# zyansheep/shadow

Hardware: AMD Instinct MI355X
Metric: APSP routing build (s) @10k nodes; packets routed/sec per sim round (lower is better)
Workload: dtype u64+f32; 1 GPU; C3 APSP routing build: 10k-node undirected ring+chords graph, mean degree 8, latency U[1,100] ms (integer us), loss 0 w.p. 0.8 else U(0,0.02); all nodes used; source rows sharded across ranks (each rank keeps its row block; the optional RCCL all-gather of the blocks is timed separately in apsp_detail.allgather_ms); nodes=10000, arcs=79996, parallelism=rows1

## Files before the change

shadow_amd/csrc/sg_routing.hip:

```cpp
#include <algorithm>
#include <cstring>
#include <string>
#include <vector>

#include "sg_device.h"
#include "sg_internal.h"
#include "sg_knobs.h"

namespace sg {

__global__ void k_self_check(const uint32_t* __restrict__ used, uint32_t n_used,
                             const uint32_t* __restrict__ self_cnt,
                             unsigned long long* __restrict__ first) {
  for (uint32_t j = blockIdx.x * blockDim.x + threadIdx.x; j < n_used; j += gridDim.x * blockDim.x) {
    uint32_t c = self_cnt[used[j]];
    if (c != 1) atomicMin(first, ((unsigned long long)j << 1) | (c > 1 ? 1ull : 0ull));
  }
}

__global__ void __launch_bounds__(1024) k_build_finish(const uint32_t* __restrict__ sat, uint32_t rows,
                                                       const uint32_t* __restrict__ used, uint32_t n_used,
                                                       const uint32_t* __restrict__ self_cnt, uint32_t* __restrict__ ret,
                                                       int count_flags) {
  constexpr int G = 8;
// ... 321 lines not shown
  for (uint32_t r = 0; r < n_diag; r++) {
    for (int k = 0; k < DW; k++) a[k] += (double)h[(size_t)r * DW + k];
    const unsigned long long w3 = h[(size_t)r * DW + 3];
    setup += (double)(w3 >> 24);
    a[3] -= (double)(w3 >> 22 << 22);
    if (h[(size_t)r * DW] == 0) continue;
    const int c = (int)((w3 >> 22) & 1);
    cn[c] += 1;
    cs[c] += (double)(w3 >> 24);
    cq[c] += (double)h[(size_t)r * DW];
  }
  for (int c = 0; c < 2; c++)
    fprintf(stderr, "[sssp] %s rows: %.0f, mean setup %.0f cyc, mean search %.0f cyc\n", c ? "chained" : "unchained",
            cn[c], cs[c] / std::max(1.0, cn[c]), cq[c] / std::max(1.0, cn[c]));
  fprintf(stderr, "[sssp] mean setup (init + bound rows) %.0f cyc of the search\n", setup / n_diag);
  fprintf(stderr, "[sssp] setup parts: bound-row listing and load issue %.0f, LDS pass %.0f, barrier %.0f, first load "
          "round %.0f, later rounds and closing barrier %.0f cyc\n", a[9] / n_diag, a[8] / n_diag, a[10] / n_diag,
          a[11] / n_diag, a[12] / n_diag);
  fprintf(stderr, "[sssp] per-wave cycles summed over a row's 16 waves: claim+wait %.0f, pop %.0f, steps %.0f "
          "(per pop: %.0f, %.0f)\n", a[5] / n_diag, a[6] / n_diag, a[7] / n_diag, a[6] / std::max(1.0, a[2]),
          a[7] / std::max(1.0, a[2]));
  fprintf(stderr, "[sssp] delta %u ns, %u rows: mean search %.0f cyc, output %.0f cyc, %.1f wave pops, %.1f buckets, "
          "%.0f relaxations (%.2f x arcs)\n", delta, n_diag, a[0] / n_diag, a[1] / n_diag, a[2] / n_diag,
          a[3] / n_diag, a[4] / n_diag, a[4] / n_diag / std::max(1u, net->n_arcs));
}

static void shortest_paths_lds(sg_ctx* ctx, sg_net* net, const uint32_t* d_used, uint32_t n_used, uint32_t row_begin,
                               uint32_t row_end, uint64_t* out_lat, float* out_loss) {
  hipStream_t st = ctx->stream;
  const uint32_t rows = row_end - row_begin;
  const LdsKnobs k = lds_knobs(ctx, net, n_used, rows);
  *(volatile uint32_t*)(ctx->apsp_ret + 4) = 0u;
  bool told = false;
// ... 484 lines not shown
```

shadow_amd/csrc/sg_sssp.hip:

```cpp
#include <algorithm>
#include <cstdlib>
#include <type_traits>

#include "sg_device.h"
#include "sg_internal.h"
#include "sg_knobs.h"

namespace sg {

constexpr int SSSP_THREADS = 1024;
constexpr int SSSP_WAVES = SSSP_THREADS / 64;
constexpr int SSSP_K = 4;
constexpr int SSSP_KB = SSSP_KB_MAX;
constexpr size_t SSSP_STATIC_LDS = 4 * (8 + SSSP_WAVES) + 16 + SSSP_WAVES * 64 * SSSP_K + 512 + 4 * (3 * SSSP_KB + 1) + 16;

constexpr size_t LDS_PER_CU = 160 * 1024;

constexpr uint64_t FKEY_INF = ((uint64_t)LAT32_SAT << 32) | ((uint64_t)0x3F800000u << 1);
__device__ __forceinline__ uint32_t fkey_lat(uint64_t k) { return (uint32_t)(k >> 32); }
__device__ __forceinline__ uint32_t fkey_loss_bits(uint64_t k) { return ((uint32_t)k >> 1) & 0x7FFFFFFFu; }
__device__ __forceinline__ uint64_t frelax(uint64_t ku, uint32_t edge_lat, float edge_om) {
  const uint32_t lat = __builtin_elementwise_add_sat(fkey_lat(ku), edge_lat);
  const float loss = fold_loss(__uint_as_float(fkey_loss_bits(ku)), edge_om);
  return ((uint64_t)lat << 32) | (uint32_t)((__float_as_uint(loss) << 1) | 1u);
// ... 89 lines not shown
    const __amdgpu_buffer_rsrc_t ro = __builtin_amdgcn_make_buffer_rsrc((void*)out_off, 0, (int)((n + 1) * 4u),
                                                                        0x00020000);
    constexpr int GO = 12;
    for (uint32_t v0 = tid; v0 <= n; v0 += GO * NT) {
      uint32_t to[GO];
#pragma unroll
      for (int g = 0; g < GO; g++) {
        const uint32_t v = v0 + g * NT;
        to[g] = __builtin_amdgcn_raw_buffer_load_b32(ro, v <= n ? v * 4u : OOB, 0, 0);
      }
#pragma unroll
      for (int g = 0; g < GO; g++)
        if (v0 + g * NT <= n) off[v0 + g * NT] = to[g];
    }
  }
  __shared__ uint32_t s_item;
  __shared__ uint32_t s_chain, s_cw, s_psat;
  auto next_listed = [&]() -> uint32_t {
    uint32_t* claim_w = chain_on ? chain_args()->claim : nullptr;
    for (;;) {
      const uint32_t b = atomicAdd(item_ctr, 1u);
      if (!claim_w || b >= n_items) return b;
      const uint32_t r = blk_rows ? blk_rows[b] : row_begin + b;
      if (atomicCAS(&claim_w[r - row_begin], 0u, 1u) == 0u) return b;
    }
  };
  for (uint32_t i = tid; i < cap; i += NT) ring[i] = RING_EMPTY;
  for (int i = tid; i < NW * 64 * SSSP_K; i += NT) (&own[0][0])[i] = 0;
  if (pop_diag && tid < SSSP_POP_WORDS) s_popc[tid] = 0ull;
  if (item_ctr && tid == 0) {
    s_item = next_listed();
    s_chain = 0u;
    s_psat = 0u;
  }
  for (uint32_t it = 0;; it++) {
    uint32_t bi, chain = 0, chain_w = 0;
    if (item_ctr) {
      __syncthreads();
      bi = s_item;
      if (bi >= n_items) break;
      if (chain_on) {
        chain = s_chain;
        chain_w = s_cw;
        if (chain > 1u && !(chain_args()->exact && !s_psat)) chain = 1u;
      }
    } else {
      if (it) break;
      bi = blockIdx.x;
      if (bi >= n_items) break;
// ... 27 lines not shown
      }
      if (lane == 0) s_nub = (uint32_t)__popcll(mk);
    };
    int nb = 0;
    if (ub_row && (FLAG ? tid < 64 : it == 0)) list_bounds(bi);
    if (ub_row) {
      if constexpr (FLAG) {
        __syncthreads();
      } else {
        __builtin_amdgcn_fence(__ATOMIC_RELEASE, "wavefront");
        __builtin_amdgcn_wave_barrier();
        __builtin_amdgcn_fence(__ATOMIC_ACQUIRE, "wavefront");
      }
      nb = (int)s_nub;
    }
    unsigned long long c_list = 0, c_init = 0, c_bar = 0, c_g0 = 0;
    auto lds_pass = [&]() {
      if (dg) c_list = clock64();
      if (chain) {
        const bool ex = (chain & 2u) != 0;
        for (uint32_t v = tid; v < n; v += NT) {
          const uint64_t kv = key[v];
          const uint64_t lw = (uint64_t)fkey_lat(kv) + chain_w;
          uint64_t nk = FKEY_INF;
          if (fkey_lat(kv) != LAT32_SAT && lw < LAT32_SAT - 1)
            nk = ex ? (lw << 32) | ((uint32_t)kv & ~1u) : ((lw + 1) << 32) | ((uint64_t)0x3F800000u << 1);
          key[v] = nk;
        }
        if (COUNT && tid == 0) {
          atomicAdd(&work[WORK_SHARDS], 1ull);
          if (ex) atomicAdd(&work[WORK_SHARDS + 1], 1ull);
        }
      } else {
        for (uint32_t v = tid; v < n; v += NT) key[v] = FKEY_INF;
      }
      if (tid < 8) ctl[tid] = 0;
      if (tid == 0) hb = 0;
      if (dg) c_init = clock64();
      __syncthreads();
      if (dg) c_bar = clock64();
    };
    if (!nb) {
      lds_pass();
    } else {
      constexpr int GC = 10;
      const __amdgpu_buffer_rsrc_t ru = __builtin_amdgcn_make_buffer_rsrc((void*)used, 0, (int)(n_used * 4u),
                                                                          0x00020000);
      int k = 0;
      uint32_t jb = 0;
      uint32_t ts = (uint32_t)tid;
      asm volatile("" : "+v"(ts));
#pragma unroll 1
      do {
        const uint32_t j0 = jb + ts;
        uint32_t vv[GC];
        uint64_t l[2][GC];
        uint32_t f[2][GC];
        bool on[2], exact[2];
        uint32_t sr[2];
#pragma unroll
        for (int u = 0; u < 2; u++) {
          on[u] = k + u < nb;
          sr[u] = on[u] ? __builtin_amdgcn_readfirstlane(s_ub[k + u][0]) : 0u;
          exact[u] = on[u] && __builtin_amdgcn_readfirstlane(s_ub[k + u][2]);
          const size_t rb = on[u] ? (size_t)(sr[u] - out_row0) * n_used : 0;
          const __amdgpu_buffer_rsrc_t rl =
              __builtin_amdgcn_make_buffer_rsrc((void*)(out_lat + rb), 0, (int)(on[u] ? n_used * 8u : 0u), 0x00020000);
          const __amdgpu_buffer_rsrc_t rf = __builtin_amdgcn_make_buffer_rsrc(
// ... 43 lines not shown
      } while (k < nb);
    }
    if (ub_row) __syncthreads();
    const unsigned long long c_setup = dg ? clock64() : 0;
    if (tid == 0) {
      key[src] = 1ull;
      ring[0] = (uint16_t)src;
      ctl[TAIL] = 1;
      s_psat = 0u;
    }
    uint32_t split = delta;
    const __amdgpu_buffer_rsrc_t arcs = __builtin_amdgcn_make_buffer_rsrc((void*)out_arc, 0, (int)(n_arcs * 12u),
                                                                          0x00020000);
    uint32_t n_rel = 0;
    const uint32_t max_adv = 4u * n + 64u;
    uint8_t* ow = own[wv];
    uint32_t spins = 0;
    constexpr int ABORT = 2;
    auto give_up = [&]() {
      if (lane == 0) {
        sat_row[row - row_begin] = 2u;
        *any_flag = 1u;
        if (atomicExch(&ctl[ABORT], 1u) == 0u && item_ctr) {
          __threadfence();
          if (atomicAdd(&item_ctr[1], 1u) == gridDim.x - 1) {
            const uint32_t c = __hip_atomic_load(&item_ctr[0], __ATOMIC_RELAXED, __HIP_MEMORY_SCOPE_AGENT);
            uint32_t* claim_w = chain_on ? chain_args()->claim : nullptr;
            for (uint32_t i = min(c, n_items); i < n_items; i++) {
              const uint32_t r = (blk_rows ? blk_rows[i] : row_begin + i) - row_begin;
              if (!claim_w || __hip_atomic_load(&claim_w[r], __ATOMIC_RELAXED, __HIP_MEMORY_SCOPE_AGENT) == 0u)
                sat_row[r] = 2u;
            }
          }
// ... 8 lines not shown
#pragma unroll
      for (int c = 0; c < NK; c++) {
        const bool ok = valid[c] && fkey_lat(cand[c]) != LAT32_SAT;
        okk[c] = ok;
        cd[c] = cand[c];
        old[c] = __hip_atomic_fetch_min(ok ? &key[v[c]] : &sink[lane], (unsigned long long)cd[c], __ATOMIC_RELAXED,
                                        __HIP_MEMORY_SCOPE_WORKGROUP);
      }
      __builtin_amdgcn_sched_barrier(0);
#pragma unroll
      for (int c = 0; c < NK; c++)
        app[c] = __builtin_amdgcn_ballot_w64(okk[c] && !((uint32_t)old[c] & 1u) && old[c] > cd[c] &&
                                             fkey_lat(cd[c]) < split);
    };
    __syncthreads();

    for (;;) {
      const unsigned long long tc0 = (COUNT && diag) ? clock64() : 0;
      uint32_t h = 0, k = 0;
      if (lane == 0) {
        for (;;) {
          const unsigned long long w = __hip_atomic_load(&hb, __ATOMIC_RELAXED, __HIP_MEMORY_SCOPE_WORKGROUP);
          const uint32_t hh = (uint32_t)(w >> 32), t = ld(&ctl[TAIL]);
          if (t == hh) break;
          const uint32_t kk = min(claim, t - hh);
          const unsigned long long nw = ((unsigned long long)(hh + kk) << 32) | ((w & 0xFFFFFFFFull) + 1);
          if (atomicCAS(&hb, w, nw) == w) {
            h = hh;
            k = kk;
            break;
          }
        }
      }
      h = __builtin_amdgcn_readfirstlane(h);
      k = __builtin_amdgcn_readfirstlane(k);
      if (__builtin_amdgcn_readfirstlane(ld(&ctl[ABORT]))) goto wave_exit;
      if (!k) {
        uint32_t q = 0;
        if (lane == 0) {
          const unsigned long long w = __hip_atomic_load(&hb, __ATOMIC_RELAXED, __HIP_MEMORY_SCOPE_WORKGROUP);
          __atomic_signal_fence(__ATOMIC_SEQ_CST);
          q = (w & 0xFFFFFFFFull) == 0 && (uint32_t)(w >> 32) == ld(&ctl[TAIL]);
        }
        if (!__builtin_amdgcn_readfirstlane(q)) {
          if (++spins > spin_max) {
            give_up();
            goto wave_exit;
          }
          for (uint32_t z = 0; z < idle_sleep; z++) __builtin_amdgcn_s_sleep(8);
          __builtin_amdgcn_s_sleep(2);
          continue;
        }
        __syncthreads();
        if (ld(&ctl[ABORT])) goto wave_exit;
        if (split >= LAT32_SAT) break;
        uint32_t m = LAT32_SAT;
        for (uint32_t v = tid; v < n; v += NT) {
          const uint64_t kv = key[v];
          if (kv & 1ull) m = min(m, fkey_lat(kv));
        }
        for (int d = 32; d > 0; d >>= 1) m = min(m, (uint32_t)__shfl_xor(m, d));
        if (lane == 0) red[wv] = m;
        __syncthreads();
        m = red[0];
        for (int w = 1; w < NW; w++) m = min(m, red[w]);
        if (m == LAT32_SAT) break;
        if (++n_adv > max_adv) {
          give_up();
          goto wave_exit;
        }
        split = m + delta >= m ? min(m + delta, LAT32_SAT) : LAT32_SAT;
        for (uint32_t v0 = wv * 64; v0 < n; v0 += NT) {
          const uint32_t v = v0 + lane;
          uint64_t kv = v < n ? key[v] : 0ull;
          const bool q2 = (kv & 1ull) && fkey_lat(kv) < split;
          const uint64_t m2 = __ballot(q2);
          append_q<1>(&m2, &v, ring, &ctl[TAIL], slot_of, lane);
        }
        __syncthreads();
        continue;
      }
      if (COUNT) n_pops++;
      const unsigned long long tc1 = (COUNT && diag) ? clock64() : 0;
      const bool on = lane < (int)k;
      uint32_t u = 0, a0 = 0, a1 = 0;
      uint64_t ku = 0;
      bool stuck = false;
      if (on) {
        uint16_t* slot = &ring[slot_of(h + lane)];
        uint16_t x;
        uint32_t sp = 0;
        while ((x = __hip_atomic_load(slot, __ATOMIC_RELAXED, __HIP_MEMORY_SCOPE_WORKGROUP)) == RING_EMPTY &&
               ++sp < spin_max)
          __builtin_amdgcn_s_sleep(0);
        stuck = x == RING_EMPTY;
        __hip_atomic_store(slot, RING_EMPTY, __ATOMIC_RELAXED, __HIP_MEMORY_SCOPE_WORKGROUP);
        u = stuck ? src : x;
        a0 = off[u];
        a1 = off[u + 1];
        ku = __hip_atomic_fetch_and(&key[u], ~1ull, __ATOMIC_RELAXED, __HIP_MEMORY_SCOPE_WORKGROUP) & ~1ull;
      }
      if (__any(stuck)) {
        give_up();
        goto wave_exit;
      }
      const uint32_t deg = a1 - a0;
      const uint32_t deg_incl = wave_incl_sum(deg);
      const uint32_t T = __builtin_amdgcn_readlane(deg_incl, 63);
      const unsigned long long tc2 = (COUNT && (diag || pop_diag)) ? clock64() : 0;
      auto expand = [&](auto kx, uint32_t ea0, uint32_t edeg, uint32_t incl) {
        constexpr int KX = decltype(kx)::value;
        const uint32_t base = incl - edeg;
        const uint32_t T = __builtin_amdgcn_readlane(incl, 63);
        if (COUNT) n_rel += T;
        uint32_t carry = 0;
        for (uint32_t t0 = 0; t0 < T; t0 += 64 * KX) {
          if (edeg && base >= t0 && base - t0 < 64u * KX) ow[base - t0] = (uint8_t)(lane + 1);
          __builtin_amdgcn_fence(__ATOMIC_RELEASE, "wavefront");
          __builtin_amdgcn_wave_barrier();
          __builtin_amdgcn_fence(__ATOMIC_ACQUIRE, "wavefront");
          uint32_t v[KX], lat[KX], om[KX], o[KX];
          bool valid[KX];
          uint64_t app[KX];
#pragma unroll
          for (int c = 0; c < KX; c++) {
            const uint32_t hd = ow[c * 64 + lane];
            ow[c * 64 + lane] = 0;
            const uint32_t mx = max(wave_incl_max(hd), carry);
            carry = __builtin_amdgcn_readlane(mx, 63);
            o[c] = mx - 1;
          }
#pragma unroll
          for (int c = 0; c < KX; c++) {
            const uint32_t sl = t0 + c * 64 + lane;
            valid[c] = sl < T;
            const uint32_t a = __shfl(ea0, (int)o[c]) + sl - __shfl(base, (int)o[c]);
            const auto r = __builtin_amdgcn_raw_buffer_load_b96(arcs, valid[c] ? a * 12u : 0x80000000u, 0, 0);
            v[c] = r[0];
            lat[c] = r[1];
            om[c] = r[2];
          }
          uint64_t cand[KX];
#pragma unroll
          for (int c = 0; c < KX; c++) {
            const uint32_t klo = __shfl((uint32_t)ku, (int)o[c]), khi = __shfl((uint32_t)(ku >> 32), (int)o[c]);
            cand[c] = frelax(((uint64_t)khi << 32) | klo, lat[c], __uint_as_float(om[c]));
          }
          offer_all(std::integral_constant<int, KX>(), valid, v, cand, app);
          append_q<KX>(app, v, ring, &ctl[TAIL], slot_of, lane);
        }
      };
      const bool small = T <= step_arcs;
      if (small && T <= 64u) {
        expand(std::integral_constant<int, 1>(), a0, deg, deg_incl);
      } else if (small && T <= 128u) {
        expand(std::integral_constant<int, 2>(), a0, deg, deg_incl);
      } else if (small || __builtin_amdgcn_ballot_w64(deg > lane_deg_max)) {
        expand(std::integral_constant<int, SSSP_K>(), a0, deg, deg_incl);
      } else {
        if (COUNT) n_rel += __builtin_amdgcn_readlane(wave_incl_sum(min(deg, (uint32_t)LA)), 63);
        if (pop_diag && lane == 0) atomicAdd(&s_popc[3 * SSSP_POP_CLASSES], 1ull);
        {
          constexpr uint32_t j0 = 0;
          uint32_t v[LA], lat[LA], om[LA];
          bool valid[LA];
          uint64_t app[LA];
#pragma unroll
          for (int c = 0; c < LA; c++) {
            valid[c] = j0 + c < deg;
            const auto r = __builtin_amdgcn_raw_buffer_load_b96(arcs, valid[c] ? (a0 + j0 + c) * 12u : 0x80000000u,
                                                                0, 0);
            v[c] = r[0];
            lat[c] = r[1];
            om[c] = r[2];
          }
          uint64_t cand[LA];
#pragma unroll
          for (int c = 0; c < LA; c++) cand[c] = frelax(ku, lat[c], __uint_as_float(om[c]));
          offer_all(std::integral_constant<int, LA>(), valid, v, cand, app);
          append_q<LA>(app, v, ring, &ctl[TAIL], slot_of, lane);
        }
        if (__builtin_amdgcn_ballot_w64(deg > (uint32_t)LA)) {
          const uint32_t rest = deg > (uint32_t)LA ? deg - LA : 0u;
          expand(std::integral_constant<int, 1>(), a0 + LA, rest, wave_incl_sum(rest));
        }
      }
      if (lane == 0) atomicSub(&hb, 1ull);
      if (COUNT && (diag || pop_diag)) {
        const unsigned long long tc3 = clock64();
        if (diag) {
          cyc_claim += tc1 - tc0;
          cyc_pop += tc2 - tc1;
          cyc_steps += tc3 - tc2;
        }
        if (pop_diag && lane == 0) {
          const uint32_t S = (T + 63u) / 64u;
          const int cls = S <= 2u ? (int)S : S <= 4u ? 3 : S <= 8u ? 4 : 5;
          atomicAdd(&s_popc[3 * cls], 1ull);
          atomicAdd(&s_popc[3 * cls + 1], (unsigned long long)T);
          atomicAdd(&s_popc[3 * cls + 2], tc3 - tc2);
        }
      }
    }
    if (COUNT && lane == 0 && n_rel) atomicAdd(&work[bi & 63], (unsigned long long)n_rel);
    if (COUNT && diag && bi < 4096 && lane == 0) {
      if (n_rel) atomicAdd(&diag[bi * SSSP_DIAG_WORDS + 4], (unsigned long long)n_rel);
      if (n_pops) atomicAdd(&diag[bi * SSSP_DIAG_WORDS + 2], (unsigned long long)n_pops);
      atomicAdd(&diag[bi * SSSP_DIAG_WORDS + 5], cyc_claim);
      atomicAdd(&diag[bi * SSSP_DIAG_WORDS + 6], cyc_pop);
      atomicAdd(&diag[bi * SSSP_DIAG_WORDS + 7], cyc_steps);
    }
    const unsigned long long c_search = dg ? clock64() : 0;
    if (COUNT) {
      uint32_t left = 0;
      for (uint32_t i = tid; i < cap; i += NT) left += ring[i] != RING_EMPTY;
      if (left) atomicAdd(&work[WORK_SHARDS + 2], (unsigned long long)left);
      if (tid == 0) atomicAdd(&work[WORK_SHARDS + 3], 1ull);
    }

    __syncthreads();
    if (pop_diag) {
      if (tid < SSSP_POP_WORDS - 1 && s_popc[tid]) {
        atomicAdd(&popc[tid], s_popc[tid]);
        s_popc[tid] = 0ull;
      }
      if (lane == 0 && n_pops) atomicAdd(&popc[SSSP_POP_WORDS - 1], (unsigned long long)n_pops);
    }
    if (item_ctr && !chain_on) {
      if (wv == 0) {
        uint32_t ni = 0;
        if (lane == 0) s_item = ni = atomicAdd(item_ctr, 1u);
        if (!FLAG && ub_row) {
          ni = __builtin_amdgcn_readfirstlane(ni);
          if (ni < n_items) list_bounds(ni);
        }
      }
    } else if (item_ctr && wv == NW - 1) {
      uint32_t ll = (uint32_t)lane;
      asm volatile("" : "+v"(ll));
      const SsspChainDesc* cd = chain_args();
      uint32_t* claim_w = cd->claim;
      const uint32_t* rel = cd->rel;
      const uint8_t* phase_of = cd->phase_of;
      const uint32_t* list_pos = cd->pos;
      const uint32_t a0 = off[src], nd = min(off[src + 1] - a0, 64u);
      const bool in = ll < nd;
      const auto r = __builtin_amdgcn_raw_buffer_load_b96(arcs, in ? (a0 + ll) * 12u : OOB, 0, 0);
      const __amdgpu_buffer_rsrc_t rr = __builtin_amdgcn_make_buffer_rsrc((void*)rel, 0, (int)(n * 4u), 0x00020000);
      const uint32_t q = __builtin_amdgcn_raw_buffer_load_b32(rr, in ? r[0] * 4u : OOB, 0, 0);
      bool ok = in && q != ~0u;
      if (const uint32_t vr = cd->check_rows) {
        const __amdgpu_buffer_rsrc_t ru = __builtin_amdgcn_make_buffer_rsrc((void*)used, 0, (int)(n_used * 4u), 0x00020000);
// ... 28 lines not shown
          break;
        }
        if (ok && q == mq) sc = ~0ull;
      }
      uint32_t ni = 0;
      if (lane == 0) {
        s_item = ni = got ? nb : next_listed();
        s_chain = cf;
        s_cw = cw;
      }
      if (ub_row) {
        ni = __builtin_amdgcn_readfirstlane(ni);
        if (ni < n_items) list_bounds(ni);
      }
    }
    const size_t orow = (size_t)(row - out_row0) * n_used;
    bool sat = false;
    typedef unsigned long long u64x2 __attribute__((ext_vector_type(2)));
    typedef float f32x4 __attribute__((ext_vector_type(4)));
    const __amdgpu_buffer_rsrc_t wl = __builtin_amdgcn_make_buffer_rsrc((void*)(out_lat + orow), 0, 0x7FFFFFFF, 0x00020000);
    const __amdgpu_buffer_rsrc_t wf = __builtin_amdgcn_make_buffer_rsrc((void*)(out_loss + orow), 0, 0x7FFFFFFF, 0x00020000);
    auto st_lat2 = [&](uint32_t j, uint64_t a, uint64_t b) {
      if constexpr (FLAG) {
        typedef uint32_t v4 __attribute__((ext_vector_type(4)));
        __builtin_amdgcn_raw_buffer_store_b128((v4){(uint32_t)a, (uint32_t)(a >> 32), (uint32_t)b, (uint32_t)(b >> 32)},
                                               wl, j * 8u, 0, SSSP_SC1);
      } else {
        __builtin_nontemporal_store((u64x2){a, b}, (u64x2*)&out_lat[orow + j]);
      }
    };
// ... 13 lines not shown
        f = e_loss[e];
      } else {
        const uint64_t kk = key[ident ? j : used[j]];
        sat |= fkey_lat(kk) == LAT32_SAT;
        l = fkey_lat(kk);
        f = __uint_as_float(fkey_loss_bits(kk));
      }
    };
    if (vec_out) {
      constexpr int OU = 4;
      const __amdgpu_buffer_rsrc_t ru = __builtin_amdgcn_make_buffer_rsrc((void*)used, 0, (int)(n_used * 4u),
                                                                          0x00020000);
      uint32_t tt = (uint32_t)tid;
      asm volatile("" : "+v"(tt));
      typedef uint32_t u32x4 __attribute__((ext_vector_type(4)));
      u32x4 uv[OU];
#pragma unroll
      for (int k = 0; k < OU; k++) {
        const uint32_t j = (tt + (uint32_t)k * NT) * 4;
        if (ident) uv[k] = (u32x4){j, j + 1, j + 2, j + 3};
        else uv[k] = __builtin_amdgcn_raw_buffer_load_b128(ru, j < n_used ? j * 4u : OOB, 0, 0);
      }
      const uint32_t de = self_edge[src];
      const uint64_t d_lat = e_lat[de];
      const float d_loss = e_loss[de];
      auto cell = [&](uint32_t j, uint32_t vj, uint64_t& l, float& f) {
        const uint64_t kk = key[vj];
        const bool diag = j == row;
        sat |= !diag && fkey_lat(kk) == LAT32_SAT;
        l = diag ? d_lat : (uint64_t)fkey_lat(kk);
        f = diag ? d_loss : __uint_as_float(fkey_loss_bits(kk));
      };
#pragma unroll
      for (int k = 0; k < OU; k++) {
        const uint32_t j = (tt + (uint32_t)k * NT) * 4;
        if (j < n_used) {
          uint64_t l0, l1, l2, l3;
          float f0, f1, f2, f3;
          cell(j, uv[k][0], l0, f0);
          cell(j + 1, uv[k][1], l1, f1);
          cell(j + 2, uv[k][2], l2, f2);
          cell(j + 3, uv[k][3], l3, f3);
          st_lat2(j, l0, l1);
          st_lat2(j + 2, l2, l3);
          st_loss4(j, f0, f1, f2, f3);
        }
      }
      for (uint32_t j = (tt + OU * NT) * 4; j < n_used; j += NT * 4) {
        uint64_t l0, l1, l2, l3;
        float f0, f1, f2, f3;
        entry(j, l0, f0);
        entry(j + 1, l1, f1);
        entry(j + 2, l2, f2);
        entry(j + 3, l3, f3);
        st_lat2(j, l0, l1);
        st_lat2(j + 2, l2, l3);
        st_loss4(j, f0, f1, f2, f3);
      }
    } else {
      for (uint32_t j = tid; j < n_used; j += NT) {
        uint64_t l;
        float f;
        entry(j, l, f);
        if constexpr (FLAG) {
          __builtin_amdgcn_raw_buffer_store_b64((uint32_t __attribute__((ext_vector_type(2)))){(uint32_t)l,
                                                                                              (uint32_t)(l >> 32)},
                                                wl, j * 8u, 0, SSSP_SC1);
          __builtin_amdgcn_raw_buffer_store_b32(__float_as_uint(f), wf, j * 4u, 0, SSSP_SC1);
        } else {
          out_lat[orow + j] = l;
          out_loss[orow + j] = f;
        }
      }
    }
    if (__any(sat) && lane == 0) {
      sat_row[row - row_begin] = 1u;
      *any_flag = 1u;
      if (FLAG) s_sat = 1u;
      if (chain_on) s_psat = 1u;
    }
    if (dg) {
      diag[bi * SSSP_DIAG_WORDS + 0] = c_search - c_start;
      diag[bi * SSSP_DIAG_WORDS + 1] = clock64() - c_search;
      diag[bi * SSSP_DIAG_WORDS + 3] = n_adv | ((unsigned long long)chain << 22) | ((c_setup - c_start) << 24);
      diag[bi * SSSP_DIAG_WORDS + 8] = c_init - c_list;
      diag[bi * SSSP_DIAG_WORDS + 9] = c_list - c_start;
      diag[bi * SSSP_DIAG_WORDS + 10] = c_bar - c_list;
      diag[bi * SSSP_DIAG_WORDS + 11] = c_g0 - c_bar;
      diag[bi * SSSP_DIAG_WORDS + 12] = c_setup - c_g0;
    }
    if constexpr (FLAG) {
      asm volatile("s_waitcnt vmcnt(0)" ::: "memory");
      __syncthreads();
      if (tid == 0) {
        const __amdgpu_buffer_rsrc_t rd = __builtin_amdgcn_make_buffer_rsrc((void*)done, 0, 0x7FFFFFFF, 0x00020000);
        __builtin_amdgcn_raw_buffer_store_b32(s_sat ? 2u : 1u, rd, (row - row_begin) * 4u, 0, SSSP_SC1);
        s_sat = 0u;
      }
    }
    __syncthreads();
  }
wave_exit:;
}
// ... 73 lines not shown
```

Baseline: 2.484 ms.

## Overlap next row's bound-row claim and loads with current row's search and output

New measurement: 2.476 ms, median of 6. No clear change (-0.3%).

```diff
diff --git a/shadow_amd/csrc/sg_routing.hip b/shadow_amd/csrc/sg_routing.hip
--- a/shadow_amd/csrc/sg_routing.hip
+++ b/shadow_amd/csrc/sg_routing.hip
@@ -359,9 +359,11 @@
     fprintf(stderr, "[sssp] %s rows: %.0f, mean setup %.0f cyc, mean search %.0f cyc\n", c ? "chained" : "unchained",
             cn[c], cs[c] / std::max(1.0, cn[c]), cq[c] / std::max(1.0, cn[c]));
   fprintf(stderr, "[sssp] mean setup (init + bound rows) %.0f cyc of the search\n", setup / n_diag);
-  fprintf(stderr, "[sssp] setup parts: bound-row listing and load issue %.0f, LDS pass %.0f, barrier %.0f, first load "
-          "round %.0f, later rounds and closing barrier %.0f cyc\n", a[9] / n_diag, a[8] / n_diag, a[10] / n_diag,
-          a[11] / n_diag, a[12] / n_diag);
+  const struct { const char* name; double cyc; } parts[] = {
+      {"early claim (its wave alone, inside the search)", a[9]}, {"next row's load issue", a[10]},
+      {"output", a[1]}, {"rewrite+merge", a[8]}, {"of which a separate LDS pass", a[11]},
+      {"later rounds and closing barrier", a[12]}};
+  for (const auto& p : parts) fprintf(stderr, "[sssp] hand-over part: %s %.0f cyc\n", p.name, p.cyc / n_diag);
   fprintf(stderr, "[sssp] per-wave cycles summed over a row's 16 waves: claim+wait %.0f, pop %.0f, steps %.0f "
           "(per pop: %.0f, %.0f)\n", a[5] / n_diag, a[6] / n_diag, a[7] / n_diag, a[6] / std::max(1.0, a[2]),
           a[7] / std::max(1.0, a[2]));
diff --git a/shadow_amd/csrc/sg_sssp.hip b/shadow_amd/csrc/sg_sssp.hip
--- a/shadow_amd/csrc/sg_sssp.hip
+++ b/shadow_amd/csrc/sg_sssp.hip
@@ -127,6 +127,7 @@
         if (v0 + g * NT <= n) off[v0 + g * NT] = to[g];
     }
   }
+  const bool early = !FLAG && item_ctr != nullptr;
   __shared__ uint32_t s_item;
   __shared__ uint32_t s_chain, s_cw, s_psat;
   auto next_listed = [&]() -> uint32_t {
@@ -146,6 +147,9 @@
     s_chain = 0u;
     s_psat = 0u;
   }
+  constexpr int GC = 10;
+  uint64_t h_l[GC];
+  uint32_t h_f[GC];
   for (uint32_t it = 0;; it++) {
     uint32_t bi, chain = 0, chain_w = 0;
     if (item_ctr) {
@@ -203,7 +207,7 @@
       }
       nb = (int)s_nub;
     }
-    unsigned long long c_list = 0, c_init = 0, c_bar = 0, c_g0 = 0;
+    unsigned long long c_list = 0, c_bar = 0, c_g0 = 0;
     auto lds_pass = [&]() {
       if (dg) c_list = clock64();
       if (chain) {
@@ -225,22 +229,102 @@
       }
       if (tid < 8) ctl[tid] = 0;
       if (tid == 0) hb = 0;
-      if (dg) c_init = clock64();
       __syncthreads();
       if (dg) c_bar = clock64();
     };
     if (!nb) {
       lds_pass();
     } else {
-      constexpr int GC = 10;
       const __amdgpu_buffer_rsrc_t ru = __builtin_amdgcn_make_buffer_rsrc((void*)used, 0, (int)(n_used * 4u),
                                                                           0x00020000);
       int k = 0;
       uint32_t jb = 0;
       uint32_t ts = (uint32_t)tid;
       asm volatile("" : "+v"(ts));
+      if constexpr (!FLAG) {
+        if (early && it > 0) {
+          const uint32_t j0 = ts;
+          uint32_t vv[GC];
+          uint64_t l1[GC];
+          uint32_t f1[GC];
+          const bool on1 = nb > 1;
+          const uint32_t sr0 = __builtin_amdgcn_readfirstlane(s_ub[0][0]);
+          const uint32_t sr1 = on1 ? __builtin_amdgcn_readfirstlane(s_ub[1][0]) : 0u;
+          const bool exact0 = __builtin_amdgcn_readfirstlane(s_ub[0][2]);
+          const bool exact1 = on1 && __builtin_amdgcn_readfirstlane(s_ub[1][2]);
+          {
+            const size_t rb = on1 ? (size_t)(sr1 - out_row0) * n_used : 0;
+            const __amdgpu_buffer_rsrc_t rl =
+                __builtin_amdgcn_make_buffer_rsrc((void*)(out_lat + rb), 0, (int)(on1 ? n_used * 8u : 0u), 0x00020000);
+            const __amdgpu_buffer_rsrc_t rf = __builtin_amdgcn_make_buffer_rsrc(
+                (void*)(out_loss + rb), 0, (int)(exact1 ? n_used * 4u : 0u), 0x00020000);
+#pragma unroll
+            for (int g = 0; g < GC; g++) {
+              const uint32_t j = j0 + g * NT;
+              const auto x = __builtin_amdgcn_raw_buffer_load_b64(rl, j < n_used ? j * 8u : OOB, 0, 0);
+              l1[g] = ((uint64_t)x[1] << 32) | x[0];
+              f1[g] = __builtin_amdgcn_raw_buffer_load_b32(rf, j < n_used ? j * 4u : OOB, 0, 0);
+            }
+          }
+          if (!ident) {
+#pragma unroll
+            for (int g = 0; g < GC; g++) {
+              const uint32_t j = j0 + g * NT;
+              vv[g] = __builtin_amdgcn_raw_buffer_load_b32(ru, j < n_used ? j * 4u : OOB, 0, 0);
+            }
+            lds_pass();
+          }
+          const bool fuse = ident != 0;
+          const bool ex = (chain & 2u) != 0;
+          auto start_key = [&](uint32_t v) -> uint64_t {
+            if (!chain) return FKEY_INF;
+            const uint64_t kv = key[v];
+            const uint64_t lw = (uint64_t)fkey_lat(kv) + chain_w;
+            if (fkey_lat(kv) == LAT32_SAT || lw >= LAT32_SAT - 1) return FKEY_INF;
+            return ex ? (lw << 32) | ((uint32_t)kv & ~1u) : ((lw + 1) << 32) | ((uint64_t)0x3F800000u << 1);
+          };
+          const uint32_t w0 = __builtin_amdgcn_readfirstlane(s_ub[0][1]);
+          const uint32_t w1 = on1 ? __builtin_amdgcn_readfirstlane(s_ub[1][1]) : 0u;
+          auto bound = [&](uint64_t kv, uint64_t lat, uint32_t fb, uint32_t w, bool exact, bool self) {
+            const uint64_t ub = lat + w;
+            if (ub < w) return kv;
+            if (ub < LAT32_SAT - 1) kv = min(kv, ((ub + 1) << 32) | ((uint64_t)0x3F800000u << 1));
+            if (exact && ub < LAT32_SAT && !self) kv = min(kv, (ub << 32) | ((uint64_t)fb << 1));
+            return kv;
+          };
+#pragma unroll
+          for (int g = 0; g < GC; g++) {
+            const uint32_t j = j0 + g * NT;
+            if (j >= n_used) {
+              if (fuse && j < n) key[j] = start_key(j);
+              continue;
+            }
+            const uint32_t v = ident ? j : vv[g];
+            const uint64_t k0 = fuse ? start_key(v) : key[v];
+            uint64_t kv = bound(k0, h_l[g], h_f[g], w0, exact0, j == sr0);
+            if (on1) kv = bound(kv, l1[g], f1[g], w1, exact1, j == sr1);
+            if (fuse || kv != k0) key[v] = kv;
+          }
+          if (fuse) {
+            for (uint32_t v = j0 + GC * NT; v < n; v += NT) key[v] = start_key(v);
+            if (COUNT && chain && tid == 0) {
+              atomicAdd(&work[WORK_SHARDS], 1ull);
+              if (ex) atomicAdd(&work[WORK_SHARDS + 1], 1ull);
+            }
+            if (tid < 8) ctl[tid] = 0;
+            if (tid == 0) hb = 0;
+          }
+          if (dg) c_g0 = clock64();
+          jb = GC * NT;
+          if (jb >= n_used) {
+            jb = 0;
+            k = 2;
+          }
+        }
+      }
+      if (k < nb)
 #pragma unroll 1
-      do {
+        do {
         const uint32_t j0 = jb + ts;
         uint32_t vv[GC];
         uint64_t l[2][GC];
@@ -314,9 +398,17 @@
                                                                           0x00020000);
     uint32_t n_rel = 0;
     const uint32_t max_adv = 4u * n + 64u;
-    uint8_t* ow = own[wv];
     uint32_t spins = 0;
     constexpr int ABORT = 2;
+    auto leave = [&]() {
+      if (early && wv == NW - 1 && lane == 0) {
+        const uint32_t ni = s_item;
+        if (ni < n_items) {
+          sat_row[(blk_rows ? blk_rows[ni] : row_begin + ni) - row_begin] = 2u;
+          *any_flag = 1u;
+        }
+      }
+    };
     auto give_up = [&]() {
       if (lane == 0) {
         sat_row[row - row_begin] = 2u;
@@ -355,228 +447,17 @@
                                              fkey_lat(cd[c]) < split);
     };
     __syncthreads();
-
-    for (;;) {
-      const unsigned long long tc0 = (COUNT && diag) ? clock64() : 0;
-      uint32_t h = 0, k = 0;
-      if (lane == 0) {
-        for (;;) {
-          const unsigned long long w = __hip_atomic_load(&hb, __ATOMIC_RELAXED, __HIP_MEMORY_SCOPE_WORKGROUP);
-          const uint32_t hh = (uint32_t)(w >> 32), t = ld(&ctl[TAIL]);
-          if (t == hh) break;
-          const uint32_t kk = min(claim, t - hh);
-          const unsigned long long nw = ((unsigned long long)(hh + kk) << 32) | ((w & 0xFFFFFFFFull) + 1);
-          if (atomicCAS(&hb, w, nw) == w) {
-            h = hh;
-            k = kk;
-            break;
-          }
-        }
-      }
-      h = __builtin_amdgcn_readfirstlane(h);
-      k = __builtin_amdgcn_readfirstlane(k);
-      if (__builtin_amdgcn_readfirstlane(ld(&ctl[ABORT]))) goto wave_exit;
-      if (!k) {
-        uint32_t q = 0;
-        if (lane == 0) {
-          const unsigned long long w = __hip_atomic_load(&hb, __ATOMIC_RELAXED, __HIP_MEMORY_SCOPE_WORKGROUP);
-          __atomic_signal_fence(__ATOMIC_SEQ_CST);
-          q = (w & 0xFFFFFFFFull) == 0 && (uint32_t)(w >> 32) == ld(&ctl[TAIL]);
-        }
-        if (!__builtin_amdgcn_readfirstlane(q)) {
-          if (++spins > spin_max) {
-            give_up();
-            goto wave_exit;
-          }
-          for (uint32_t z = 0; z < idle_sleep; z++) __builtin_amdgcn_s_sleep(8);
-          __builtin_amdgcn_s_sleep(2);
-          continue;
-        }
-        __syncthreads();
-        if (ld(&ctl[ABORT])) goto wave_exit;
-        if (split >= LAT32_SAT) break;
-        uint32_t m = LAT32_SAT;
-        for (uint32_t v = tid; v < n; v += NT) {
-          const uint64_t kv = key[v];
-          if (kv & 1ull) m = min(m, fkey_lat(kv));
-        }
-        for (int d = 32; d > 0; d >>= 1) m = min(m, (uint32_t)__shfl_xor(m, d));
-        if (lane == 0) red[wv] = m;
-        __syncthreads();
-        m = red[0];
-        for (int w = 1; w < NW; w++) m = min(m, red[w]);
-        if (m == LAT32_SAT) break;
-        if (++n_adv > max_adv) {
-          give_up();
-          goto wave_exit;
-        }
-        split = m + delta >= m ? min(m + delta, LAT32_SAT) : LAT32_SAT;
-        for (uint32_t v0 = wv * 64; v0 < n; v0 += NT) {
-          const uint32_t v = v0 + lane;
-          uint64_t kv = v < n ? key[v] : 0ull;
-          const bool q2 = (kv & 1ull) && fkey_lat(kv) < split;
-          const uint64_t m2 = __ballot(q2);
-          append_q<1>(&m2, &v, ring, &ctl[TAIL], slot_of, lane);
-        }
-        __syncthreads();
-        continue;
-      }
-      if (COUNT) n_pops++;
-      const unsigned long long tc1 = (COUNT && diag) ? clock64() : 0;
-      const bool on = lane < (int)k;
-      uint32_t u = 0, a0 = 0, a1 = 0;
-      uint64_t ku = 0;
-      bool stuck = false;
-      if (on) {
-        uint16_t* slot = &ring[slot_of(h + lane)];
-        uint16_t x;
-        uint32_t sp = 0;
-        while ((x = __hip_atomic_load(slot, __ATOMIC_RELAXED, __HIP_MEMORY_SCOPE_WORKGROUP)) == RING_EMPTY &&
-               ++sp < spin_max)
-          __builtin_amdgcn_s_sleep(0);
-        stuck = x == RING_EMPTY;
-        __hip_atomic_store(slot, RING_EMPTY, __ATOMIC_RELAXED, __HIP_MEMORY_SCOPE_WORKGROUP);
-        u = stuck ? src : x;
-        a0 = off[u];
-        a1 = off[u + 1];
-        ku = __hip_atomic_fetch_and(&key[u], ~1ull, __ATOMIC_RELAXED, __HIP_MEMORY_SCOPE_WORKGROUP) & ~1ull;
-      }
-      if (__any(stuck)) {
-        give_up();
-        goto wave_exit;
-      }
-      const uint32_t deg = a1 - a0;
-      const uint32_t deg_incl = wave_incl_sum(deg);
-      const uint32_t T = __builtin_amdgcn_readlane(deg_incl, 63);
-      const unsigned long long tc2 = (COUNT && (diag || pop_diag)) ? clock64() : 0;
-      auto expand = [&](auto kx, uint32_t ea0, uint32_t edeg, uint32_t incl) {
-        constexpr int KX = decltype(kx)::value;
-        const uint32_t base = incl - edeg;
-        const uint32_t T = __builtin_amdgcn_readlane(incl, 63);
-        if (COUNT) n_rel += T;
-        uint32_t carry = 0;
-        for (uint32_t t0 = 0; t0 < T; t0 += 64 * KX) {
-          if (edeg && base >= t0 && base - t0 < 64u * KX) ow[base - t0] = (uint8_t)(lane + 1);
-          __builtin_amdgcn_fence(__ATOMIC_RELEASE, "wavefront");
-          __builtin_amdgcn_wave_barrier();
-          __builtin_amdgcn_fence(__ATOMIC_ACQUIRE, "wavefront");
-          uint32_t v[KX], lat[KX], om[KX], o[KX];
-          bool valid[KX];
-          uint64_t app[KX];
-#pragma unroll
-          for (int c = 0; c < KX; c++) {
-            const uint32_t hd = ow[c * 64 + lane];
-            ow[c * 64 + lane] = 0;
-            const uint32_t mx = max(wave_incl_max(hd), carry);
-            carry = __builtin_amdgcn_readlane(mx, 63);
-            o[c] = mx - 1;
-          }
-#pragma unroll
-          for (int c = 0; c < KX; c++) {
-            const uint32_t sl = t0 + c * 64 + lane;
-            valid[c] = sl < T;
-            const uint32_t a = __shfl(ea0, (int)o[c]) + sl - __shfl(base, (int)o[c]);
-            const auto r = __builtin_amdgcn_raw_buffer_load_b96(arcs, valid[c] ? a * 12u : 0x80000000u, 0, 0);
-            v[c] = r[0];
-            lat[c] = r[1];
-            om[c] = r[2];
-          }
-          uint64_t cand[KX];
-#pragma unroll
-          for (int c = 0; c < KX; c++) {
-            const uint32_t klo = __shfl((uint32_t)ku, (int)o[c]), khi = __shfl((uint32_t)(ku >> 32), (int)o[c]);
-            cand[c] = frelax(((uint64_t)khi << 32) | klo, lat[c], __uint_as_float(om[c]));
-          }
-          offer_all(std::integral_constant<int, KX>(), valid, v, cand, app);
-          append_q<KX>(app, v, ring, &ctl[TAIL], slot_of, lane);
-        }
-      };
-      const bool small = T <= step_arcs;
-      if (small && T <= 64u) {
-        expand(std::integral_constant<int, 1>(), a0, deg, deg_incl);
-      } else if (small && T <= 128u) {
-        expand(std::integral_constant<int, 2>(), a0, deg, deg_incl);
-      } else if (small || __builtin_amdgcn_ballot_w64(deg > lane_deg_max)) {
-        expand(std::integral_constant<int, SSSP_K>(), a0, deg, deg_incl);
-      } else {
-        if (COUNT) n_rel += __builtin_amdgcn_readlane(wave_incl_sum(min(deg, (uint32_t)LA)), 63);
-        if (pop_diag && lane == 0) atomicAdd(&s_popc[3 * SSSP_POP_CLASSES], 1ull);
-        {
-          constexpr uint32_t j0 = 0;
-          uint32_t v[LA], lat[LA], om[LA];
-          bool valid[LA];
-          uint64_t app[LA];
-#pragma unroll
-          for (int c = 0; c < LA; c++) {
-            valid[c] = j0 + c < deg;
-            const auto r = __builtin_amdgcn_raw_buffer_load_b96(arcs, valid[c] ? (a0 + j0 + c) * 12u : 0x80000000u,
-                                                                0, 0);
-            v[c] = r[0];
-            lat[c] = r[1];
-            om[c] = r[2];
-          }
-          uint64_t cand[LA];
-#pragma unroll
-          for (int c = 0; c < LA; c++) cand[c] = frelax(ku, lat[c], __uint_as_float(om[c]));
-          offer_all(std::integral_constant<int, LA>(), valid, v, cand, app);
-          append_q<LA>(app, v, ring, &ctl[TAIL], slot_of, lane);
-        }
-        if (__builtin_amdgcn_ballot_w64(deg > (uint32_t)LA)) {
-          const uint32_t rest = deg > (uint32_t)LA ? deg - LA : 0u;
-          expand(std::integral_constant<int, 1>(), a0 + LA, rest, wave_incl_sum(rest));
-        }
-      }
-      if (lane == 0) atomicSub(&hb, 1ull);
-      if (COUNT && (diag || pop_diag)) {
-        const unsigned long long tc3 = clock64();
-        if (diag) {
-          cyc_claim += tc1 - tc0;
-          cyc_pop += tc2 - tc1;
-          cyc_steps += tc3 - tc2;
-        }
-        if (pop_diag && lane == 0) {
-          const uint32_t S = (T + 63u) / 64u;
-          const int cls = S <= 2u ? (int)S : S <= 4u ? 3 : S <= 8u ? 4 : 5;
-          atomicAdd(&s_popc[3 * cls], 1ull);
-          atomicAdd(&s_popc[3 * cls + 1], (unsigned long long)T);
-          atomicAdd(&s_popc[3 * cls + 2], tc3 - tc2);
-        }
-      }
-    }
-    if (COUNT && lane == 0 && n_rel) atomicAdd(&work[bi & 63], (unsigned long long)n_rel);
-    if (COUNT && diag && bi < 4096 && lane == 0) {
-      if (n_rel) atomicAdd(&diag[bi * SSSP_DIAG_WORDS + 4], (unsigned long long)n_rel);
-      if (n_pops) atomicAdd(&diag[bi * SSSP_DIAG_WORDS + 2], (unsigned long long)n_pops);
-      atomicAdd(&diag[bi * SSSP_DIAG_WORDS + 5], cyc_claim);
-      atomicAdd(&diag[bi * SSSP_DIAG_WORDS + 6], cyc_pop);
-      atomicAdd(&diag[bi * SSSP_DIAG_WORDS + 7], cyc_steps);
-    }
-    const unsigned long long c_search = dg ? clock64() : 0;
-    if (COUNT) {
-      uint32_t left = 0;
-      for (uint32_t i = tid; i < cap; i += NT) left += ring[i] != RING_EMPTY;
-      if (left) atomicAdd(&work[WORK_SHARDS + 2], (unsigned long long)left);
-      if (tid == 0) atomicAdd(&work[WORK_SHARDS + 3], 1ull);
-    }
-
-    __syncthreads();
-    if (pop_diag) {
-      if (tid < SSSP_POP_WORDS - 1 && s_popc[tid]) {
-        atomicAdd(&popc[tid], s_popc[tid]);
-        s_popc[tid] = 0ull;
-      }
-      if (lane == 0 && n_pops) atomicAdd(&popc[SSSP_POP_WORDS - 1], (unsigned long long)n_pops);
-    }
-    if (item_ctr && !chain_on) {
-      if (wv == 0) {
+    const unsigned long long c_claim0 = (COUNT && diag && early && wv == NW - 1) ? clock64() : 0;
+    if (early && !chain_on) {
+      if (wv == NW - 1) {
         uint32_t ni = 0;
         if (lane == 0) s_item = ni = atomicAdd(item_ctr, 1u);
-        if (!FLAG && ub_row) {
+        if (ub_row) {
           ni = __builtin_amdgcn_readfirstlane(ni);
           if (ni < n_items) list_bounds(ni);
         }
       }
-    } else if (item_ctr && wv == NW - 1) {
+    } else if (early && wv == NW - 1) {
       uint32_t ll = (uint32_t)lane;
       asm volatile("" : "+v"(ll));
       const SsspChainDesc* cd = chain_args();
@@ -635,6 +516,258 @@
         if (ni < n_items) list_bounds(ni);
       }
     }
+    if (COUNT && diag && early && tid == NT - 64 && bi < 4096)
+      diag[bi * SSSP_DIAG_WORDS + 9] = clock64() - c_claim0;
+
+    uint32_t tid_s = (uint32_t)threadIdx.x;
+    asm volatile("" : "+v"(tid_s));
+    {
+    const int lane = (int)(tid_s & 63u), wv = (int)(tid_s >> 6);
+    uint8_t* ow = own[wv];
+    for (;;) {
+      const unsigned long long tc0 = (COUNT && diag) ? clock64() : 0;
+      uint32_t h = 0, k = 0;
+      if (lane == 0) {
+        for (;;) {
+          const unsigned long long w = __hip_atomic_load(&hb, __ATOMIC_RELAXED, __HIP_MEMORY_SCOPE_WORKGROUP);
+          const uint32_t hh = (uint32_t)(w >> 32), t = ld(&ctl[TAIL]);
+          if (t == hh) break;
+          const uint32_t kk = min(claim, t - hh);
+          const unsigned long long nw = ((unsigned long long)(hh + kk) << 32) | ((w & 0xFFFFFFFFull) + 1);
+          if (atomicCAS(&hb, w, nw) == w) {
+            h = hh;
+            k = kk;
+            break;
+          }
+        }
+      }
+      h = __builtin_amdgcn_readfirstlane(h);
+      k = __builtin_amdgcn_readfirstlane(k);
+      if (__builtin_amdgcn_readfirstlane(ld(&ctl[ABORT]))) {
+        leave();
+        goto wave_exit;
+      }
+      if (!k) {
+        uint32_t q = 0;
+        if (lane == 0) {
+          const unsigned long long w = __hip_atomic_load(&hb, __ATOMIC_RELAXED, __HIP_MEMORY_SCOPE_WORKGROUP);
+          __atomic_signal_fence(__ATOMIC_SEQ_CST);
+          q = (w & 0xFFFFFFFFull) == 0 && (uint32_t)(w >> 32) == ld(&ctl[TAIL]);
+        }
+        if (!__builtin_amdgcn_readfirstlane(q)) {
+          if (++spins > spin_max) {
+            give_up();
+            leave();
+            goto wave_exit;
+          }
+          for (uint32_t z = 0; z < idle_sleep; z++) __builtin_amdgcn_s_sleep(8);
+          __builtin_amdgcn_s_sleep(2);
+          continue;
+        }
+        __syncthreads();
+        if (ld(&ctl[ABORT])) {
+          leave();
+          goto wave_exit;
+        }
+        if (split >= LAT32_SAT) break;
+        uint32_t m = LAT32_SAT;
+        for (uint32_t v = tid; v < n; v += NT) {
+          const uint64_t kv = key[v];
+          if (kv & 1ull) m = min(m, fkey_lat(kv));
+        }
+        for (int d = 32; d > 0; d >>= 1) m = min(m, (uint32_t)__shfl_xor(m, d));
+        if (lane == 0) red[wv] = m;
+        __syncthreads();
+        m = red[0];
+        for (int w = 1; w < NW; w++) m = min(m, red[w]);
+        if (m == LAT32_SAT) break;
+        if (++n_adv > max_adv) {
+          give_up();
+          leave();
+          goto wave_exit;
+        }
+        split = m + delta >= m ? min(m + delta, LAT32_SAT) : LAT32_SAT;
+        for (uint32_t v0 = wv * 64; v0 < n; v0 += NT) {
+          const uint32_t v = v0 + lane;
+          uint64_t kv = v < n ? key[v] : 0ull;
+          const bool q2 = (kv & 1ull) && fkey_lat(kv) < split;
+          const uint64_t m2 = __ballot(q2);
+          append_q<1>(&m2, &v, ring, &ctl[TAIL], slot_of, lane);
+        }
+        __syncthreads();
+        continue;
+      }
+      if (COUNT) n_pops++;
+      const unsigned long long tc1 = (COUNT && diag) ? clock64() : 0;
+      const bool on = lane < (int)k;
+      uint32_t u = 0, a0 = 0, a1 = 0;
+      uint64_t ku = 0;
+      bool stuck = false;
+      if (on) {
+        uint16_t* slot = &ring[slot_of(h + lane)];
+        uint16_t x;
+        uint32_t sp = 0;
+        while ((x = __hip_atomic_load(slot, __ATOMIC_RELAXED, __HIP_MEMORY_SCOPE_WORKGROUP)) == RING_EMPTY &&
+               ++sp < spin_max)
+          __builtin_amdgcn_s_sleep(0);
+        stuck = x == RING_EMPTY;
+        __hip_atomic_store(slot, RING_EMPTY, __ATOMIC_RELAXED, __HIP_MEMORY_SCOPE_WORKGROUP);
+        u = stuck ? src : x;
+        a0 = off[u];
+        a1 = off[u + 1];
+        ku = __hip_atomic_fetch_and(&key[u], ~1ull, __ATOMIC_RELAXED, __HIP_MEMORY_SCOPE_WORKGROUP) & ~1ull;
+      }
+      if (__any(stuck)) {
+        give_up();
+        leave();
+        goto wave_exit;
+      }
+      const uint32_t deg = a1 - a0;
+      const uint32_t deg_incl = wave_incl_sum(deg);
+      const uint32_t T = __builtin_amdgcn_readlane(deg_incl, 63);
+      const unsigned long long tc2 = (COUNT && (diag || pop_diag)) ? clock64() : 0;
+      auto expand = [&](auto kx, uint32_t ea0, uint32_t edeg, uint32_t incl) {
+        constexpr int KX = decltype(kx)::value;
+        const uint32_t base = incl - edeg;
+        const uint32_t T = __builtin_amdgcn_readlane(incl, 63);
+        if (COUNT) n_rel += T;
+        uint32_t carry = 0;
+        for (uint32_t t0 = 0; t0 < T; t0 += 64 * KX) {
+          if (edeg && base >= t0 && base - t0 < 64u * KX) ow[base - t0] = (uint8_t)(lane + 1);
+          __builtin_amdgcn_fence(__ATOMIC_RELEASE, "wavefront");
+          __builtin_amdgcn_wave_barrier();
+          __builtin_amdgcn_fence(__ATOMIC_ACQUIRE, "wavefront");
+          uint32_t v[KX], lat[KX], om[KX], o[KX];
+          bool valid[KX];
+          uint64_t app[KX];
+#pragma unroll
+          for (int c = 0; c < KX; c++) {
+            const uint32_t hd = ow[c * 64 + lane];
+            ow[c * 64 + lane] = 0;
+            const uint32_t mx = max(wave_incl_max(hd), carry);
+            carry = __builtin_amdgcn_readlane(mx, 63);
+            o[c] = mx - 1;
+          }
+#pragma unroll
+          for (int c = 0; c < KX; c++) {
+            const uint32_t sl = t0 + c * 64 + lane;
+            valid[c] = sl < T;
+            const uint32_t a = __shfl(ea0, (int)o[c]) + sl - __shfl(base, (int)o[c]);
+            const auto r = __builtin_amdgcn_raw_buffer_load_b96(arcs, valid[c] ? a * 12u : 0x80000000u, 0, 0);
+            v[c] = r[0];
+            lat[c] = r[1];
+            om[c] = r[2];
+          }
+          uint64_t cand[KX];
+#pragma unroll
+          for (int c = 0; c < KX; c++) {
+            const uint32_t klo = __shfl((uint32_t)ku, (int)o[c]), khi = __shfl((uint32_t)(ku >> 32), (int)o[c]);
+            cand[c] = frelax(((uint64_t)khi << 32) | klo, lat[c], __uint_as_float(om[c]));
+          }
+          offer_all(std::integral_constant<int, KX>(), valid, v, cand, app);
+          append_q<KX>(app, v, ring, &ctl[TAIL], slot_of, lane);
+        }
+      };
+      const bool small = T <= step_arcs;
+      if (small && T <= 64u) {
+        expand(std::integral_constant<int, 1>(), a0, deg, deg_incl);
+      } else if (small && T <= 128u) {
+        expand(std::integral_constant<int, 2>(), a0, deg, deg_incl);
+      } else if (small || __builtin_amdgcn_ballot_w64(deg > lane_deg_max)) {
+        expand(std::integral_constant<int, SSSP_K>(), a0, deg, deg_incl);
+      } else {
+        if (COUNT) n_rel += __builtin_amdgcn_readlane(wave_incl_sum(min(deg, (uint32_t)LA)), 63);
+        if (pop_diag && lane == 0) atomicAdd(&s_popc[3 * SSSP_POP_CLASSES], 1ull);
+        {
+          constexpr uint32_t j0 = 0;
+          uint32_t v[LA], lat[LA], om[LA];
+          bool valid[LA];
+          uint64_t app[LA];
+#pragma unroll
+          for (int c = 0; c < LA; c++) {
+            valid[c] = j0 + c < deg;
+            const auto r = __builtin_amdgcn_raw_buffer_load_b96(arcs, valid[c] ? (a0 + j0 + c) * 12u : 0x80000000u,
+                                                                0, 0);
+            v[c] = r[0];
+            lat[c] = r[1];
+            om[c] = r[2];
+          }
+          uint64_t cand[LA];
+#pragma unroll
+          for (int c = 0; c < LA; c++) cand[c] = frelax(ku, lat[c], __uint_as_float(om[c]));
+          offer_all(std::integral_constant<int, LA>(), valid, v, cand, app);
+          append_q<LA>(app, v, ring, &ctl[TAIL], slot_of, lane);
+        }
+        if (__builtin_amdgcn_ballot_w64(deg > (uint32_t)LA)) {
+          const uint32_t rest = deg > (uint32_t)LA ? deg - LA : 0u;
+          expand(std::integral_constant<int, 1>(), a0 + LA, rest, wave_incl_sum(rest));
+        }
+      }
+      if (lane == 0) atomicSub(&hb, 1ull);
+      if (COUNT && (diag || pop_diag)) {
+        const unsigned long long tc3 = clock64();
+        if (diag) {
+          cyc_claim += tc1 - tc0;
+          cyc_pop += tc2 - tc1;
+          cyc_steps += tc3 - tc2;
+        }
+        if (pop_diag && lane == 0) {
+          const uint32_t S = (T + 63u) / 64u;
+          const int cls = S <= 2u ? (int)S : S <= 4u ? 3 : S <= 8u ? 4 : 5;
+          atomicAdd(&s_popc[3 * cls], 1ull);
+          atomicAdd(&s_popc[3 * cls + 1], (unsigned long long)T);
+          atomicAdd(&s_popc[3 * cls + 2], tc3 - tc2);
+        }
+      }
+    }
+    }
+    if (COUNT && lane == 0 && n_rel) atomicAdd(&work[bi & 63], (unsigned long long)n_rel);
+    if (COUNT && diag && bi < 4096 && lane == 0) {
+      if (n_rel) atomicAdd(&diag[bi * SSSP_DIAG_WORDS + 4], (unsigned long long)n_rel);
+      if (n_pops) atomicAdd(&diag[bi * SSSP_DIAG_WORDS + 2], (unsigned long long)n_pops);
+      atomicAdd(&diag[bi * SSSP_DIAG_WORDS + 5], cyc_claim);
+      atomicAdd(&diag[bi * SSSP_DIAG_WORDS + 6], cyc_pop);
+      atomicAdd(&diag[bi * SSSP_DIAG_WORDS + 7], cyc_steps);
+    }
+    const unsigned long long c_search = dg ? clock64() : 0;
+    if (COUNT) {
+      uint32_t left = 0;
+      for (uint32_t i = tid; i < cap; i += NT) left += ring[i] != RING_EMPTY;
+      if (left) atomicAdd(&work[WORK_SHARDS + 2], (unsigned long long)left);
+      if (tid == 0) atomicAdd(&work[WORK_SHARDS + 3], 1ull);
+    }
+
+    __syncthreads();
+    if (pop_diag) {
+      if (tid < SSSP_POP_WORDS - 1 && s_popc[tid]) {
+        atomicAdd(&popc[tid], s_popc[tid]);
+        s_popc[tid] = 0ull;
+      }
+      if (lane == 0 && n_pops) atomicAdd(&popc[SSSP_POP_WORDS - 1], (unsigned long long)n_pops);
+    }
+    if (FLAG && item_ctr && tid == 0) s_item = atomicAdd(item_ctr, 1u);
+    const unsigned long long c_issue = dg ? clock64() : 0;
+    unsigned long long c_out = c_issue;
+    auto issue_held = [&]() __attribute__((always_inline)) {
+      const bool on0 = early && ub_row && s_item < n_items && s_nub;
+      const uint32_t sr0 = on0 ? __builtin_amdgcn_readfirstlane(s_ub[0][0]) : 0u;
+      const bool exact0 = on0 && __builtin_amdgcn_readfirstlane(s_ub[0][2]);
+      const size_t rb = on0 ? (size_t)(sr0 - out_row0) * n_used : 0;
+      const __amdgpu_buffer_rsrc_t rl =
+          __builtin_amdgcn_make_buffer_rsrc((void*)(out_lat + rb), 0, (int)(on0 ? n_used * 8u : 0u), 0x00020000);
+      const __amdgpu_buffer_rsrc_t rf =
+          __builtin_amdgcn_make_buffer_rsrc((void*)(out_loss + rb), 0, (int)(exact0 ? n_used * 4u : 0u), 0x00020000);
+      uint32_t ts = (uint32_t)tid;
+      asm volatile("" : "+v"(ts));
+#pragma unroll
+      for (int g = 0; g < GC; g++) {
+        const uint32_t j = ts + g * NT;
+        const auto x = __builtin_amdgcn_raw_buffer_load_b64(rl, j < n_used ? j * 8u : OOB, 0, 0);
+        h_l[g] = ((uint64_t)x[1] << 32) | x[0];
+        h_f[g] = __builtin_amdgcn_raw_buffer_load_b32(rf, j < n_used ? j * 4u : OOB, 0, 0);
+      }
+      if (dg) c_out = clock64();
+    };
     const size_t orow = (size_t)(row - out_row0) * n_used;
     bool sat = false;
     typedef unsigned long long u64x2 __attribute__((ext_vector_type(2)));
@@ -678,37 +811,47 @@
       uint32_t tt = (uint32_t)tid;
       asm volatile("" : "+v"(tt));
       typedef uint32_t u32x4 __attribute__((ext_vector_type(4)));
-      u32x4 uv[OU];
-#pragma unroll
-      for (int k = 0; k < OU; k++) {
-        const uint32_t j = (tt + (uint32_t)k * NT) * 4;
-        if (ident) uv[k] = (u32x4){j, j + 1, j + 2, j + 3};
-        else uv[k] = __builtin_amdgcn_raw_buffer_load_b128(ru, j < n_used ? j * 4u : OOB, 0, 0);
-      }
-      const uint32_t de = self_edge[src];
-      const uint64_t d_lat = e_lat[de];
-      const float d_loss = e_loss[de];
-      auto cell = [&](uint32_t j, uint32_t vj, uint64_t& l, float& f) {
-        const uint64_t kk = key[vj];
-        const bool diag = j == row;
-        sat |= !diag && fkey_lat(kk) == LAT32_SAT;
-        l = diag ? d_lat : (uint64_t)fkey_lat(kk);
-        f = diag ? d_loss : __uint_as_float(fkey_loss_bits(kk));
+      auto out_groups = [&](auto id_t) __attribute__((always_inline)) {
+        constexpr int ID = decltype(id_t)::value;
+        u32x4 uv[OU];
+#pragma unroll
+        for (int k = 0; k < OU; k++) {
+          const uint32_t j = (tt + (uint32_t)k * NT) * 4;
+          if (ID == 1 || (ID == 2 && ident)) uv[k] = (u32x4){j, j + 1, j + 2, j + 3};
+          else uv[k] = __builtin_amdgcn_raw_buffer_load_b128(ru, j < n_used ? j * 4u : OOB, 0, 0);
+        }
+        const uint32_t de = self_edge[FLAG ? src : __builtin_amdgcn_readfirstlane(src)];
+        const uint64_t d_lat = e_lat[de];
+        const float d_loss = e_loss[de];
+        if constexpr (!FLAG) issue_held();
+        auto cell = [&](uint32_t j, uint32_t vj, uint64_t& l, float& f) {
+          const uint64_t kk = key[vj];
+          const bool diag = j == row;
+          sat |= !diag && fkey_lat(kk) == LAT32_SAT;
+          l = diag ? d_lat : (uint64_t)fkey_lat(kk);
+          f = diag ? d_loss : __uint_as_float(fkey_loss_bits(kk));
+        };
+#pragma unroll
+        for (int k = 0; k < OU; k++) {
+          const uint32_t j = (tt + (uint32_t)k * NT) * 4;
+          if (j < n_used) {
+            uint64_t l0, l1, l2, l3;
+            float f0, f1, f2, f3;
+            cell(j, uv[k][0], l0, f0);
+            cell(j + 1, uv[k][1], l1, f1);
+            cell(j + 2, uv[k][2], l2, f2);
+            cell(j + 3, uv[k][3], l3, f3);
+            st_lat2(j, l0, l1);
+            st_lat2(j + 2, l2, l3);
+            st_loss4(j, f0, f1, f2, f3);
+          }
+        }
       };
-#pragma unroll
-      for (int k = 0; k < OU; k++) {
-        const uint32_t j = (tt + (uint32_t)k * NT) * 4;
-        if (j < n_used) {
-          uint64_t l0, l1, l2, l3;
-          float f0, f1, f2, f3;
-          cell(j, uv[k][0], l0, f0);
-          cell(j + 1, uv[k][1], l1, f1);
-          cell(j + 2, uv[k][2], l2, f2);
-          cell(j + 3, uv[k][3], l3, f3);
-          st_lat2(j, l0, l1);
-          st_lat2(j + 2, l2, l3);
-          st_loss4(j, f0, f1, f2, f3);
-        }
+      if constexpr (FLAG) {
+        out_groups(std::integral_constant<int, 2>());
+      } else {
+        if (ident) out_groups(std::integral_constant<int, 1>());
+        else out_groups(std::integral_constant<int, 0>());
       }
       for (uint32_t j = (tt + OU * NT) * 4; j < n_used; j += NT * 4) {
         uint64_t l0, l1, l2, l3;
@@ -722,6 +865,7 @@
         st_loss4(j, f0, f1, f2, f3);
       }
     } else {
+      if constexpr (!FLAG) issue_held();
       for (uint32_t j = tid; j < n_used; j += NT) {
         uint64_t l;
         float f;
@@ -745,12 +889,11 @@
     }
     if (dg) {
       diag[bi * SSSP_DIAG_WORDS + 0] = c_search - c_start;
-      diag[bi * SSSP_DIAG_WORDS + 1] = clock64() - c_search;
+      diag[bi * SSSP_DIAG_WORDS + 1] = clock64() - c_out;
       diag[bi * SSSP_DIAG_WORDS + 3] = n_adv | ((unsigned long long)chain << 22) | ((c_setup - c_start) << 24);
-      diag[bi * SSSP_DIAG_WORDS + 8] = c_init - c_list;
-      diag[bi * SSSP_DIAG_WORDS + 9] = c_list - c_start;
-      diag[bi * SSSP_DIAG_WORDS + 10] = c_bar - c_list;
-      diag[bi * SSSP_DIAG_WORDS + 11] = c_g0 - c_bar;
+      diag[bi * SSSP_DIAG_WORDS + 8] = c_g0 - c_start;
+      diag[bi * SSSP_DIAG_WORDS + 10] = c_out - c_issue;
+      diag[bi * SSSP_DIAG_WORDS + 11] = c_bar - c_list;
       diag[bi * SSSP_DIAG_WORDS + 12] = c_setup - c_g0;
     }
     if constexpr (FLAG) {
```
